# XMUDM/SPEX

Measured on AMD Instinct MI355X. Metric: graph-conv edges/sec + BPR-triples/sec, LightGCN-SPEX Epinion2 d=64, higher is better.
Workload: dtype f32

## Files before the change

### include/spex_hip.h

```cpp
#ifndef SPEX_HIP_H
#define SPEX_HIP_H

#include <stdint.h>

#ifdef __cplusplus
extern "C" {
#endif

typedef enum spex_status {
    SPEX_OK = 0,
    SPEX_ERR_INVALID = -1,
    SPEX_ERR_HIP = -2,
    SPEX_ERR_COMM = -3,
    SPEX_ERR_UNSUPPORTED = -4
} spex_status;

typedef struct spex_graph spex_graph_t;

int spex_version(void);
const char *spex_last_error(void);

int spex_graph_create(const int32_t *h_rowptr, const int32_t *h_col, const float *h_val, const int32_t *h_edge_id,
                      int32_t n_rows, int32_t n_cols, int64_t nnz, spex_graph_t **out);
int spex_graph_destroy(spex_graph_t *g);
int spex_graph_pack_digest(const int32_t *h_rowptr, const int32_t *h_col, const float *h_val, int32_t n_rows, int32_t n_cols,
                           int64_t nnz, uint64_t *digest );
int spex_graph_pack_hub_table(const int32_t *h_rowptr, const int32_t *h_col, const float *h_val, int32_t n_rows, int32_t n_cols,
                              int64_t nnz, int32_t *out, int64_t cap, int64_t *n_out);
int spex_graph_pack_row_heads(const int32_t *h_rowptr, const int32_t *h_col, const float *h_val, int32_t n_rows, int32_t n_cols,
                              int64_t nnz, int32_t *out_col, float *out_val, int64_t cap, int64_t *n_out, int32_t *stride);
int spex_graph_info(const spex_graph_t *g, int32_t *n_rows, int32_t *n_cols, int64_t *nnz, int32_t *n_long_rows,
                    int32_t *n_segments);

int spex_graph_set_edge_mask(spex_graph_t *g, int mode , const uint8_t *d_keep,
                             float keep_prob, uint64_t seed);

int spex_spmm_f32(const spex_graph_t *g, const float *X, float *Y, const float *add_in, float add_div,
                  const float *acc_in, float *acc_out, float acc_div, int32_t d, void *stream);

int spex_spmm_rowlist_f32(const spex_graph_t *g, const float *X, const int64_t *idx_a, int32_t n_a, int64_t off_a,
                          const int64_t *idx_b, int32_t n_b, int64_t off_b, float *Y, const float *acc_in, float *acc_out,
                          float acc_div, int32_t d, void *stream);
int spex_spmm_owned_rows_f32(const spex_graph_t *g, const float *X, const int64_t *pos, int32_t n, int64_t lo, const float *acc_in,
                             const float *acc2, const float *acc3, float acc_div, const float *raw, float *out_prop, float *out_raw,
                             int32_t d, void *stream);

int spex_propagate_f32(const spex_graph_t *g, const float *E0, float *mean_out, float *layers_out, float *ws,
                       int32_t L, int32_t d, void *stream);

int spex_propagate_bwd_f32(const spex_graph_t *gt, const float *g_out, float *grad_E0, float *ws, int32_t L,
                           int32_t d, void *stream);

int spex_cast_bf16_f32(const float *X, uint16_t *X16, int64_t n, void *stream);

int spex_spmm_bf16_f32(const spex_graph_t *g, const uint16_t *X16, float *Y, uint16_t *Y16, const float *add_in, float add_div,
// ... 430 lines not shown
```

### spex_amd/_lib.py

```python
import ctypes
import os

_HERE = os.path.dirname(os.path.abspath(__file__))
LIB_PATH = os.path.join(_HERE, "lib", "libspexhip.so")

c_i32, c_i64, c_f32, c_vp = ctypes.c_int32, ctypes.c_int64, ctypes.c_float, ctypes.c_void_p

SIGNATURES = {
    "spex_version": (ctypes.c_int, []),
    "spex_last_error": (ctypes.c_char_p, []),
    "spex_graph_create": (ctypes.c_int, [c_vp, c_vp, c_vp, c_vp, c_i32, c_i32, c_i64, ctypes.POINTER(c_vp)]),
    "spex_graph_destroy": (ctypes.c_int, [c_vp]),
    "spex_graph_pack_digest": (ctypes.c_int, [c_vp, c_vp, c_vp, c_i32, c_i32, c_i64, c_vp]),
    "spex_graph_pack_hub_table": (ctypes.c_int, [c_vp, c_vp, c_vp, c_i32, c_i32, c_i64, c_vp, c_i64, c_vp]),
    "spex_graph_pack_row_heads": (ctypes.c_int, [c_vp, c_vp, c_vp, c_i32, c_i32, c_i64, c_vp, c_vp, c_i64, c_vp, c_vp]),
    "spex_graph_info": (ctypes.c_int, [c_vp, ctypes.POINTER(c_i32), ctypes.POINTER(c_i32), ctypes.POINTER(c_i64),
                                       ctypes.POINTER(c_i32), ctypes.POINTER(c_i32)]),
    "spex_graph_set_edge_mask": (ctypes.c_int, [c_vp, ctypes.c_int, c_vp, c_f32, ctypes.c_uint64]),
    "spex_spmm_f32": (ctypes.c_int, [c_vp, c_vp, c_vp, c_vp, c_f32, c_vp, c_vp, c_f32, c_i32, c_vp]),
    "spex_spmm_rowlist_f32": (ctypes.c_int, [c_vp, c_vp, c_vp, c_i32, c_i64, c_vp, c_i32, c_i64, c_vp, c_vp, c_vp, c_f32, c_i32,
                                             c_vp]),
    "spex_spmm_owned_rows_f32": (ctypes.c_int, [c_vp, c_vp, c_vp, c_i32, c_i64, c_vp, c_vp, c_vp, c_f32, c_vp, c_vp, c_vp, c_i32, c_vp]),
    "spex_propagate_f32": (ctypes.c_int, [c_vp, c_vp, c_vp, c_vp, c_vp, c_i32, c_i32, c_vp]),
    "spex_propagate_bwd_f32": (ctypes.c_int, [c_vp, c_vp, c_vp, c_vp, c_i32, c_i32, c_vp]),
    "spex_cast_bf16_f32": (ctypes.c_int, [c_vp, c_vp, c_i64, c_vp]),
    "spex_spmm_bf16_f32": (ctypes.c_int, [c_vp, c_vp, c_vp, c_vp, c_vp, c_f32, c_vp, c_vp, c_f32, c_i32, c_vp]),
    "spex_propagate_bf16_f32": (ctypes.c_int, [c_vp, c_vp, c_vp, c_vp, c_i32, c_i32, c_vp]),
    "spex_propagate_bwd_bf16_f32": (ctypes.c_int, [c_vp, c_vp, c_vp, c_vp, c_vp, c_i32, c_i32, c_vp]),
    "spex_score_bce_f32": (ctypes.c_int, [c_vp, c_vp, c_i32, c_i32, c_i64, c_i64, c_vp, c_vp, c_vp, c_i32, c_i32, c_vp,
                                          c_vp, c_vp, c_vp, c_f32, c_vp]),
    "spex_score_bce_slots_f32": (ctypes.c_int, [c_vp, c_vp, c_i32, c_i32, c_i64, c_i64, c_vp, c_vp, c_vp, c_i32, c_i32, c_vp, c_vp,
                                                c_vp, c_f32, c_vp, c_i32, c_vp]),
    "spex_bpr_sgd_step_f32": (ctypes.c_int, [c_vp, c_vp, c_vp, c_vp, c_i64, c_i64, c_vp, c_vp, c_vp, c_i64, c_i32,
                                             c_f32, c_f32, c_vp, c_vp]),
    "spex_bpr_loss_f32": (ctypes.c_int, [c_vp, c_vp, c_i64, c_i64, c_vp, c_vp, c_vp, c_i64, c_i32, c_vp, c_vp, c_vp,
                                         c_f32, c_vp]),
    "spex_bpr_grouped_workspace_bytes": (c_i64, [c_i64, c_i64, c_i64]),
    "spex_bpr_sgd_step_grouped_f32": (ctypes.c_int, [c_vp, c_vp, c_vp, c_vp, c_i64, c_i64, c_vp, c_vp, c_vp, c_i64, c_i32,
                                                     c_f32, c_f32, c_vp, c_vp, c_i64, c_vp]),
    "spex_bpr_loss_grouped_f32": (ctypes.c_int, [c_vp, c_vp, c_i64, c_i64, c_vp, c_vp, c_vp, c_i64, c_i32, c_vp, c_vp, c_vp,
# ... 253 lines not shown
```

### spex_amd/csrc/graph.hip

```cpp
#include <stdarg.h>
#include <stdio.h>

#include <stdlib.h>

#include <algorithm>
#include <string>
#include <thread>
#include <vector>

#include "spex_common.h"

namespace spex {
static thread_local char g_err[512] = "";
void set_error(const char *fmt, ...)
{
    va_list ap;
    va_start(ap, fmt);
    vsnprintf(g_err, sizeof(g_err), fmt, ap);
    va_end(ap);
}
}

extern "C" int spex_version(void) { return 5; }
extern "C" const char *spex_last_error(void) { return spex::g_err; }
// ... 177 lines not shown
            long_seg0.push_back((int32_t)seg_beg.size());
            for (int32_t s = b; s < e; s += spex::kSegLen) {
                seg_beg.push_back(s);
                seg_end.push_back(s + spex::kSegLen < e ? s + spex::kSegLen : e);
            }
        }
    }
    long_seg0.push_back((int32_t)seg_beg.size());
    g->n_long = (int32_t)long_row.size();
    g->n_seg = (int32_t)seg_beg.size();

    std::vector<int4> task;
    std::vector<uint32_t> c_off, c_mask, c_eid;
    std::vector<uint8_t> c_pad;
    std::vector<int32_t> c_row;
    std::vector<float> c_val;
    std::vector<int32_t> hub_row, hub_seg0;
    std::vector<int4> hub_grp;
    std::vector<int2> hub_fold;
    const bool chunked = true;
    const char *implied_sw = getenv("SPEX_PACK_IMPLIED");
    const bool pack_implied = !(implied_sw && implied_sw[0] == '0');
    g->row_ids = (int64_t)n_cols * 256 <= ((int64_t)16 << 20);
    (void)flags;
    const int32_t tile_rows = 0;
    std::vector<int32_t> wg_rows;
    constexpr int kResidentWgs = 512;
    int open_tasks_now = spex::kOpenTasks;
    int pack_cap = spex::kTaskEntries;
    bool final_pass = false;
    for (int attempt = 0; chunked && attempt < 12; ++attempt) {
        task.clear();
        wg_rows.clear();
        hub_row.clear();
        hub_seg0.clear();
        hub_grp.clear();
        hub_fold.clear();
        struct ChunkJob { int64_t first_chunk; int64_t rows_off; int32_t n_rows, b, e, r0; };
        std::vector<ChunkJob> jobs;
        std::vector<int32_t> pack_rows;
        int64_t n_planned = 0;
        jobs.reserve((size_t)nnz / 48 + 64);
        pack_rows.reserve((size_t)n_rows + 64);
        auto add_chunks = [&](const int32_t *rows, int32_t n_rows_in, int32_t b, int32_t e, int32_t r0) -> int2 {
            int64_t entries = 0;
            ChunkJob j{n_planned, (int64_t)pack_rows.size(), 0, b, e, r0};
// ... 26 lines not shown
            for (const int4 &t : task)
                if (t.y > stride) return;
            std::vector<int64_t> moved(jobs.size(), -1);
            for (size_t k = 0; k < task.size(); ++k) {
                int4 &t = task[k];
                if (t.y > 0) {
                    const size_t j = (size_t)(std::lower_bound(jobs.begin(), jobs.end(), (int64_t)t.x,
                                                               [](const ChunkJob &jb, int64_t v) { return jb.first_chunk < v; }) - jobs.begin());
                    moved[j] = (int64_t)k * stride;
                }
                t.x = (int32_t)((int64_t)k * stride);
            }
            for (size_t j = 0; j < jobs.size(); ++j) jobs[j].first_chunk = moved[j];
            n_planned = (int64_t)task.size() * stride;
            implied = true;
            g->chunk_stride = stride;
        };
        auto fill_chunks = [&]() {
            place_implied();
            const size_t n_slots = (size_t)n_planned * spex::kChunk;
            c_off.resize(n_slots);
            c_val.resize(n_slots);
            c_eid.resize(n_slots);
            if (g->row_ids) c_row.resize(n_slots);
            c_mask.resize((size_t)n_planned);
            c_pad.assign((size_t)n_planned, implied ? (uint8_t)spex::kChunk : (uint8_t)0);
            const bool row_ids = g->row_ids;
            auto fill_job = [&](const ChunkJob &j) {
                size_t pos = (size_t)j.first_chunk * spex::kChunk, ci = (size_t)j.first_chunk;
                int32_t in_chunk = 0, last_col = 0, last_eid = 0, last_row = j.r0;
                uint32_t mask = 0;
                auto put = [&](int32_t en, int32_t r, bool last) {
                    last_col = h_col[en];
                    last_eid = h_edge_id ? h_edge_id[en] : en;
                    last_row = r;
                    c_off[pos] = (uint32_t)last_col;
                    c_val[pos] = h_val[en];
                    c_eid[pos] = (uint32_t)last_eid;
                    if (row_ids) c_row[pos] = r;
                    ++pos;
                    if (last) mask |= 1u << in_chunk;
                    if (++in_chunk == spex::kChunk) {
                        c_mask[ci] = mask;
                        c_pad[ci++] = 0;
                        mask = 0;
                        in_chunk = 0;
                    }
                };
                if (j.n_rows < 0) {
                    const int32_t n = -j.n_rows, nch = (n + spex::kChunk - 1) / spex::kChunk;
                    for (int32_t k = 0; k < nch * spex::kChunk; ++k, ++pos) {
                        c_off[pos] = 0u;
                        c_val[pos] = 0.0f;
                        c_eid[pos] = 0u;
                        if (row_ids) c_row[pos] = pack_rows[(size_t)j.rows_off + (k < n ? k : n - 1)];
                    }
                    for (int32_t c = 0; c < nch; ++c) {
                        c_mask[ci + c] = 0u;
                        c_pad[ci + c] = (uint8_t)spex::kChunk;
                    }
                    return;
                }
                if (j.n_rows) {
                    for (int32_t i = 0; i < j.n_rows; ++i) {
                        const int32_t r = pack_rows[(size_t)j.rows_off + i];
                        for (int32_t en = h_rowptr[r]; en < h_rowptr[r + 1]; ++en) put(en, r, en + 1 == h_rowptr[r + 1]);
                    }
                } else {
                    for (int32_t en = j.b; en < j.e; ++en) put(en, j.r0, false);
                }
                if (in_chunk) {
                    const uint32_t n_pad = (uint32_t)(spex::kChunk - in_chunk);
                    for (; in_chunk < spex::kChunk; ++in_chunk, ++pos) {
                        c_off[pos] = (uint32_t)last_col;
                        c_val[pos] = 0.0f;
                        c_eid[pos] = (uint32_t)last_eid;
                        if (row_ids) c_row[pos] = last_row;
                    }
                    c_mask[ci] = mask;
                    c_pad[ci] = (uint8_t)n_pad;
                }
            };
            std::vector<size_t> cut((size_t)n_thr + 1, jobs.size());
            cut[0] = 0;
            for (int p = 1; p < n_thr; ++p) {
                const int64_t want = n_planned * p / n_thr;
                if (implied) {
                    cut[p] = jobs.size() * (size_t)p / (size_t)n_thr;
                    continue;
                }
                cut[p] = (size_t)(std::lower_bound(jobs.begin(), jobs.end(), want,
                                                   [](const ChunkJob &j, int64_t v) { return j.first_chunk < v; }) - jobs.begin());
            }
            parallel_parts(n_thr, [&](int p) {
                for (size_t k = cut[p]; k < cut[p + 1]; ++k) fill_job(jobs[k]);
            });
        };
// ... 154 lines not shown
    }
    g->n_tasks = (int32_t)task.size();
    g->tile_rows = tile_rows;
    g->n_wgs = (int32_t)wg_rows.size();
    std::vector<int32_t> head_col;
    std::vector<float> head_val;
    {
        const char *heads_sw = getenv("SPEX_ROW_HEADS");
        const bool wanted = !digest || head_col_dump;
        if (wanted && g->row_ids && hub_row.empty() && nnz > 0 && !(heads_sw && heads_sw[0] == '0')) {
            head_col.assign((size_t)n_rows * spex::kRowHead, 0);
            head_val.assign((size_t)n_rows * spex::kRowHead, 0.0f);
            parallel_parts(n_thr, [&](int p) {
                const int32_t r_lo = (int32_t)((int64_t)n_rows * p / n_thr), r_hi = (int32_t)((int64_t)n_rows * (p + 1) / n_thr);
                for (int32_t r = r_lo; r < r_hi; ++r) {
                    const int32_t b = h_rowptr[r], n = std::min(h_rowptr[r + 1] - b, (int32_t)spex::kRowHead);
                    std::copy(h_col + b, h_col + b + n, head_col.begin() + (size_t)r * spex::kRowHead);
                    std::copy(h_val + b, h_val + b + n, head_val.begin() + (size_t)r * spex::kRowHead);
                }
            });
        }
    }
    if (getenv("SPEX_DEBUG_PACK"))
        fprintf(stderr, "[spex] graph %d x %d nnz %lld: %d tasks = %d workgroups, %lld chunks (%.1f %% padding), tile mode %d (%d workgroups), chunk stride %d, chunk table %lld bytes, row heads %lld bytes\n",
                n_rows, n_cols, (long long)nnz, (int)task.size(), (int)task.size() / spex::kWgWaves, (long long)c_mask.size(),
                nnz ? 100.0 * ((double)c_mask.size() * spex::kChunk - (double)nnz) / (double)nnz : 0.0, tile_rows, g->n_wgs, g->chunk_stride,
                (long long)(c_off.size() * 4 + c_val.size() * 4 + c_eid.size() * 4 + c_row.size() * 4 + c_mask.size() * 4 + c_pad.size()),
                (long long)(head_col.size() * 4 + head_val.size() * 4));
    g->n_chunks = (int64_t)c_mask.size();
    g->n_hub = (int32_t)hub_row.size();
    g->n_hub_tasks = (int32_t)hub_grp.size();

    g->tile = (nnz / spex::kSoftmaxTile < 2048) ? 512 : spex::kSoftmaxTile;
    g->n_tiles = (int32_t)((nnz + g->tile - 1) / g->tile);
    std::vector<int32_t> tile_row((size_t)g->n_tiles + 1);
    {
        int32_t r = 0;
        for (int32_t t = 0; t <= g->n_tiles; ++t) {
            const int64_t first = (int64_t)t * g->tile;
            while (r < n_rows && (int64_t)h_rowptr[r] < first) ++r;
            tile_row[t] = r;
        }
    }

    if (digest) {
        if (hub_dump) {
            hub_dump->clear();
            hub_dump->push_back((int32_t)hub_grp.size());
            hub_dump->push_back((int32_t)hub_fold.size());
            for (size_t k = 0; k < hub_grp.size(); ++k) {
                const int4 t = task[k], q = hub_grp[k];
// ... 56 lines not shown
        hipError_t e = hipMalloc((void **)&g->partial, (size_t)g->partial_cap * sizeof(float));
        if (e != hipSuccess) {
            spex::set_error("hipMalloc(partial) failed: %s", hipGetErrorString(e));
            spex_graph_destroy(g);
            return SPEX_ERR_HIP;
        }
    }
    *out = g;
    return SPEX_OK;
}

extern "C" int spex_graph_info(const spex_graph_t *g, int32_t *n_rows, int32_t *n_cols, int64_t *nnz,
                               int32_t *n_long_rows, int32_t *n_segments)
{
    SPEX_CHECK_ARG(g, "spex_graph_info: NULL handle");
    if (n_rows) *n_rows = g->n_rows;
    if (n_cols) *n_cols = g->n_cols;
    if (nnz) *nnz = g->nnz;
    if (n_long_rows) *n_long_rows = g->n_long;
    if (n_segments) *n_segments = g->n_seg;
    return SPEX_OK;
}

extern "C" int spex_graph_set_edge_mask(spex_graph_t *g, int mode, const uint8_t *d_keep, float keep_prob,
                                        uint64_t seed)
{
    SPEX_CHECK_ARG(g, "spex_graph_set_edge_mask: NULL handle");
    SPEX_CHECK_ARG(mode >= 0 && mode <= 2, "spex_graph_set_edge_mask: mode %d not in {0,1,2}", mode);
    SPEX_CHECK_ARG(mode != 1 || d_keep, "spex_graph_set_edge_mask: injected mode needs a device mask");
    SPEX_CHECK_ARG(mode == 0 || (keep_prob > 0.0f), "spex_graph_set_edge_mask: keep_prob must be > 0");
    if (mode != 0 && keep_prob >= 1.0f && mode == 2) mode = 0;
    g->mask_mode = mode;
    g->keep = (mode == 1) ? d_keep : nullptr;
    g->keep_prob = keep_prob;
    g->seed = seed;
    return SPEX_OK;
}

extern "C" int spex_timer_create(int32_t capacity, int32_t every, spex_timer_t **out)
{
    SPEX_CHECK_ARG(out && capacity > 0 && capacity <= (1 << 20), "spex_timer_create: bad capacity %d", capacity);
    SPEX_CHECK_ARG(every >= 1, "spex_timer_create: every = %d", every);
    spex_timer *t = new spex_timer();
    t->every = every;
    t->start.resize(capacity);
    t->stop.resize(capacity);
// ... 45 lines not shown
```

### spex_amd/csrc/spex_common.h

```cpp
#pragma once
#include <hip/hip_runtime.h>
#include <stdint.h>
#include <mutex>
#include <string>
#include <vector>

#include "../../include/spex_hip.h"

namespace spex {

void set_error(const char *fmt, ...);
struct SmallAdam {
    float *p = nullptr, *m = nullptr, *v = nullptr;
    const float *parts = nullptr;
    int32_t n_parts = 0;
    int64_t stride = 0;
    int32_t n = 0;
};
struct L2Rows {
    const int32_t *count = nullptr;
    int32_t *clear = nullptr;
    float scale = 0.0f;
    float *g_store = nullptr;
    int32_t shift = 4;
// ... 280 lines not shown
    int32_t *seg_end = nullptr;
    int32_t *long_row = nullptr;
    int32_t *long_seg0 = nullptr;
    float *partial = nullptr;
    int64_t partial_cap = 0;
    float *snap = nullptr;
    int64_t snap_cap = 0;
    unsigned long long *loss_cell = nullptr;
    int64_t loss_cell_cap = 0;
    std::mutex scratch_mu;
    hipStream_t scratch_stream = nullptr;
    bool scratch_used = false;
    hipEvent_t scratch_ev = nullptr;
    int32_t n_tasks = 0;
    int4 *task = nullptr;
    int64_t n_chunks = 0;
    uint32_t *chunk_off = nullptr;
    float *chunk_val = nullptr;
    uint32_t *chunk_mask = nullptr;
    uint8_t *chunk_pad = nullptr;
    uint32_t *chunk_eid = nullptr;
    bool row_ids = false;
    int32_t *chunk_row = nullptr;
    int32_t chunk_stride = 0;
    int32_t *head_col = nullptr;
    float *head_val = nullptr;
    int32_t tile_rows = 0;
    int32_t n_wgs = 0;
    int32_t *wg_rows = nullptr;
    int32_t n_hub = 0;
    int32_t *hub_row = nullptr;
    int32_t *hub_seg0 = nullptr;
    int32_t n_hub_tasks = 0;
    int4 *hub_grp = nullptr;
    int2 *hub_fold = nullptr;
    unsigned long long *hub_ticket = nullptr;
    int mask_mode = 0;
    const uint8_t *keep = nullptr;
    float keep_prob = 1.0f;
    uint64_t seed = 0;
    spex_timer *timer = nullptr;
};
```

### spex_amd/csrc/spmm.hip

```cpp
#include <mutex>

#include "spmm_chunk.h"

using namespace spex;
using namespace spex::chunkk;

namespace {

struct SpmmParams {
    const int32_t *rowptr, *col;
    const float *val;
    const int32_t *edge_id;
    const int32_t *seg_beg, *seg_end, *long_row, *long_seg0;
    int32_t n_rows, n_seg, n_long;

    const float *X;
    float *Y;
    const float *add_in;
    float add_div;
    float out_div;
    const float *acc_in;
    float *acc_out;
    float acc_div;
    float *partial;
// ... 147 lines not shown
template <int V>
struct VecOf {
    typedef float T __attribute__((ext_vector_type(V)));
};

template <int EPI, bool MASKED, bool ROWIDS, int V>
__global__ __launch_bounds__(kWave *kWgWaves) void spmm_chunk_wide_kernel(
    const float *__restrict__ X, const uint32_t *__restrict__ chunk_off, const float *__restrict__ chunk_val,
    const uint32_t *__restrict__ chunk_mask, const int32_t *__restrict__ chunk_row, const int4 *__restrict__ task,
    int n_tasks, float *__restrict__ Y,
    const float *epi_in, float epi_div, float out_div, float *acc_out,
    float *__restrict__ partial,
    const DropArgs drop, const int xcd_contiguous)
{
    typedef typename VecOf<V>::T vec;
    constexpr int kRow = kWave * V;
    constexpr int kBatch = kChunk / V;
    __shared__ float s_part[kWgWaves][kRow];
    const int lane = threadIdx.x & (kWave - 1);
    const int wave = __builtin_amdgcn_readfirstlane((int)(threadIdx.x >> 6));
    const int wg = xcd_contiguous ? xcd_contiguous_block(blockIdx.x, gridDim.x) : (int)blockIdx.x;
    const int tid = wg * kWgWaves + wave;
    if (tid >= n_tasks) return;
    const int4 t = task[tid];
    const int kind = t.w & 3;
    const float *__restrict__ Xl = X + lane * V;
    const float *El = (EPI ? epi_in : X) + lane * V;
    int row = t.z;
    vec acc = (vec)(0.0f);

    auto emit = [&](int r, vec y, vec e) {
        const size_t o = (size_t)r * kRow + lane * V;
        if (EPI == 0) {
            __builtin_nontemporal_store(y, reinterpret_cast<vec *>(Y + o));
        } else if (EPI == 1) {
            if (Y) __builtin_nontemporal_store(y, reinterpret_cast<vec *>(Y + o));
            vec s = e + y;
            if (epi_div != 1.0f) s = s / epi_div;
            __builtin_nontemporal_store(s, reinterpret_cast<vec *>(acc_out + o));
        } else {
            if (epi_div != 1.0f) e = e / epi_div;
            vec s = y + e;
            if (out_div != 1.0f) s = s / out_div;
            __builtin_nontemporal_store(s, reinterpret_cast<vec *>(Y + o));
        }
    };

    const int n_ch = kind == 3 ? 0 : t.y;
    for (int sc = 0; sc < n_ch; sc += 4) {
        const int nc = (n_ch - sc < 4) ? n_ch - sc : 4;
        uint32_t my_off = 0u, my_mask = 0u, own_off = 0u;
        unsigned long long drop_bits = 0ull;
        int my_row = 0;
        float my_val = 0.0f;
        if (lane < nc * kChunk) {
            const size_t e = (size_t)(t.x + sc) * kChunk + lane;
            my_off = __builtin_nontemporal_load(chunk_off + e);
            my_val = __builtin_nontemporal_load(chunk_val + e);
            if (ROWIDS) my_row = __builtin_nontemporal_load(chunk_row + e);
            if (MASKED) own_off = drop_lane(drop, __builtin_nontemporal_load(drop.chunk_eid + e), my_val, my_off);
        }
        if (MASKED) drop_bits = drop_stand_in(lane < nc * kChunk, own_off, my_off);
        if (lane < nc) my_mask = __builtin_nontemporal_load(chunk_mask + t.x + sc + lane);
        for (int c = 0; c < nc; ++c) {
            const uint32_t mask = (uint32_t)__builtin_amdgcn_readlane((int)my_mask, c);
            const uint32_t dbits = MASKED ? (uint32_t)(drop_bits >> (c * kChunk)) & 0xFFFFu : 0u;
#pragma unroll
            for (int u0 = 0; u0 < kChunk; u0 += kBatch) {
                vec x[kBatch], ep[kBatch];
#pragma unroll
                for (int u = 0; u < kBatch; ++u)
                    x[u] = *reinterpret_cast<const vec *>(
                        Xl + (size_t)(uint32_t)__builtin_amdgcn_readlane((int)my_off, c * kChunk + u0 + u) * kRow);
                const uint32_t bmask = (mask >> u0) & ((1u << kBatch) - 1u);
                if (EPI != 0 && bmask != 0u) {
                    int r = row;
#pragma unroll
                    for (int u = 0; u < kBatch; ++u) {
                        ep[u] = (vec)(0.0f);
                        if (bmask & (1u << u)) {
                            const int rr = ROWIDS ? __builtin_amdgcn_readlane(my_row, c * kChunk + u0 + u) : r;
                            ep[u] = __builtin_nontemporal_load(reinterpret_cast<const vec *>(El + (size_t)rr * kRow));
                            ++r;
                        }
                    }
                } else {
// ... 2 lines not shown
                }
#pragma unroll
                for (int u = 0; u < kBatch; ++u) {
                    const float a = lane_bcast(my_val, c * kChunk + u0 + u);
                    const bool gone = MASKED && (dbits & (1u << (u0 + u)));
#pragma unroll
                    for (int j = 0; j < V; ++j) acc[j] = fmaf(a, gone ? 0.0f : x[u][j], acc[j]);
                    if (bmask & (1u << u)) {
                        emit(ROWIDS ? __builtin_amdgcn_readlane(my_row, c * kChunk + u0 + u) : row, acc, ep[u]);
                        acc = (vec)(0.0f);
                        ++row;
                    }
                }
            }
        }
    }
    if (kind == 0 && t.y == 0 && t.z >= 0) {
        vec e = (vec)(0.0f);
        if (EPI != 0) e = *reinterpret_cast<const vec *>(El + (size_t)t.z * kRow);
        emit(t.z, (vec)(0.0f), e);
    }
    if (ROWIDS && kind == 3) {
        const int count = t.w >> 4;
        const int my_r = lane < count ? chunk_row[(size_t)t.x * kChunk + lane] : 0;
        for (int k0 = 0; k0 < count; k0 += kBatch) {
            vec e[kBatch];
#pragma unroll
            for (int u = 0; u < kBatch; ++u) {
                e[u] = (vec)(0.0f);
                if (EPI != 0 && k0 + u < count) e[u] = *reinterpret_cast<const vec *>(El + (size_t)__builtin_amdgcn_readlane(my_r, (k0 + u) & 63) * kRow);
            }
#pragma unroll
            for (int u = 0; u < kBatch; ++u)
                if (k0 + u < count) emit(__builtin_amdgcn_readlane(my_r, (k0 + u) & 63), (vec)(0.0f), e[u]);
        }
    }
    if (kind == 2) {
#pragma unroll
        for (int j = 0; j < V; ++j) partial[(size_t)(t.w >> 4) * kRow + lane * V + j] = acc[j];
    }
    if (t.w & 4) {
        const bool leader = kind == 1 && (t.w & 8);
        const int slot = (t.w >> 4) & 15, nseg = (t.w >> 8) & 31;
        vec e = (vec)(0.0f);
        if (leader && EPI != 0) e = *reinterpret_cast<const vec *>(El + (size_t)t.z * kRow);
        if (kind == 1 && !leader) {
#pragma unroll
// ... 334 lines not shown
    const int per_block = fast ? kWgWaves : kWavesPerBlock;
    const int64_t tasks = fast ? (int64_t)g->n_tasks : (int64_t)g->n_seg + g->n_rows;
    int64_t blocks = (tasks + per_block - 1) / per_block;
    blocks = (blocks + 7) / 8 * 8;
    SnapArgs sa{nullptr, nullptr, nullptr, nullptr, 0, 0, 0, (int32_t)blocks};
    int64_t tail = 0;
    if (snap) {
        SPEX_CHECK_ARG(fast && d == 64 && !masked && !acc_out && !add_in && snap->out && snap->T > 0, "launch_spmm: the snapshot tail rides on the plain d == 64 launch only");
        sa = *snap;
        sa.table_wgs = (int32_t)blocks;
        tail = (3 * snap->T + (int64_t)kWgWaves * kWave - 1) / ((int64_t)kWgWaves * kWave);
    }
    const dim3 grid((unsigned)(blocks + tail)), block(kWave * per_block), block4(kWave * kWavesPerBlock);
    spex_timer *tm = g->timer;
    if (tm && tm->open) tm->launches[tm->used]++;
    std::unique_lock<std::mutex> scratch_lock;
    if ((fast ? g->n_hub > 0 : g->n_long > 0) || snap) {
        const int rc = order_scratch(g, stream, scratch_lock);
        if (rc) return rc;
    }
    if (fast) {
        SPEX_CHECK_ARG(((((uintptr_t)X) | ((uintptr_t)Y) | ((uintptr_t)add_in) | ((uintptr_t)acc_in) | ((uintptr_t)acc_out)) & 15) == 0,
                       "spex_spmm_f32: X / Y / add_in / acc_in / acc_out must be 16-byte aligned");
        const int xcd_contig = ((int64_t)g->n_cols * d * 4 <= (int64_t)16 << 20) ? 1 : 0;
        const DropArgs da = drop_args(g);
        const char *fold_sw = g->n_hub > 0 ? getenv("SPEX_HUB_FOLD") : nullptr;
        const bool fold_env = !(fold_sw && fold_sw[0] == '0');
        hub.grp = g->hub_grp; hub.fold = g->hub_fold; hub.ticket = g->hub_ticket;
        hub.tag = (d == 64 && fold_env && g->n_hub > 0 && g->hub_grp && g->hub_ticket) ? 1u : 0u;
        if (acc_out) launch_chunk<1>(d, masked, g->row_ids, grid, block, stream, X, g, Y, acc_in, acc_div, 1.0f, acc_out, da, xcd_contig, hub, sa);
        else if (add_in) launch_chunk<2>(d, masked, g->row_ids, grid, block, stream, X, g, Y, add_in, add_div, out_div, nullptr, da, xcd_contig, hub, sa);
        else launch_chunk<0>(d, masked, g->row_ids, grid, block, stream, X, g, Y, nullptr, 1.0f, 1.0f, nullptr, da, xcd_contig, hub, sa);
    } else if (masked) {
        hipLaunchKernelGGL((spmm_rows_kernel<true>), grid, block, 0, stream, p);
    } else {
        hipLaunchKernelGGL((spmm_rows_kernel<false>), grid, block, 0, stream, p);
    }
    if (fast) {
        if (g->n_hub > 0 && hub.tag == 0u) {
            const dim3 fgrid((unsigned)((g->n_hub + kWavesPerBlock - 1) / kWavesPerBlock));
            hipLaunchKernelGGL(spmm_long_fixup_kernel, fgrid, block4, 0, stream, p, g->hub_row, g->hub_seg0, g->hub_seg0 + 1, 2,
                               g->n_hub);
        }
    } else if (g->n_long > 0) {
        const dim3 fgrid((unsigned)((g->n_long + kWavesPerBlock - 1) / kWavesPerBlock));
        hipLaunchKernelGGL(spmm_long_fixup_kernel, fgrid, block4, 0, stream, p, g->long_row, g->long_seg0, g->long_seg0 + 1, 1,
// ... 262 lines not shown
```

### spex_amd/csrc/spmm_bf16.hip

```cpp
#include <mutex>

#include "spmm_chunk.h"

using namespace spex;
using namespace spex::chunkk;

namespace {

template <int EPI, bool MASKED, bool ROWIDS>
__global__ __launch_bounds__(kWave *kWgWaves) __attribute__((amdgpu_waves_per_eu(8, 8))) void spmm_chunk_bf16_kernel(
    const uint16_t *__restrict__ X16, const uint32_t *__restrict__ chunk_off, const float *__restrict__ chunk_val,
    const uint32_t *__restrict__ chunk_mask, const int32_t *__restrict__ chunk_row, const int4 *__restrict__ task,
    int n_tasks, float *__restrict__ Y, uint16_t *__restrict__ Y16,
    const float *epi_in, float epi_div, float *acc_out,
    float *__restrict__ partial, const DropArgs drop, const int xcd_contiguous, const int chunk_stride)
{
    chunk_body<uint16_t, EPI, MASKED, ROWIDS, false>(chunk_off, chunk_val, chunk_row, chunk_mask, task, n_tasks, xcd_contiguous, chunk_stride,
                                                     0, X16, Y, ChunkSide<uint16_t>{Y16}, epi_in, epi_div, acc_out, partial, drop,
                                                     HubFold{nullptr, nullptr, nullptr, 0u}, SnapArgs{});
}


__global__ __launch_bounds__(kWave *kWavesPerBlock) void spmm_hub_fixup_bf16_kernel(
    const float *__restrict__ partial, const int32_t *__restrict__ rows, const int32_t *__restrict__ seg, int n_hub,
// ... 65 lines not shown
    hipLaunchKernelGGL((spmm_chunk_bf16_kernel<EPI, M, R>), grid, block, 0, stream, X16, g->chunk_off, g->chunk_val, g->chunk_mask, \
                       g->chunk_row, g->task, g->n_tasks, Y, Y16, epi_in, epi_div, acc_out, g->partial, da, xcd_contig, g->chunk_stride)
    if (masked) {
        if (row_ids) SPEX_GO(true, true);
        else SPEX_GO(true, false);
    } else {
        if (row_ids) SPEX_GO(false, true);
        else SPEX_GO(false, false);
    }
#undef SPEX_GO
}

int launch_spmm_bf16(const spex_graph *g, const uint16_t *X16, float *Y, uint16_t *Y16, const float *add_in, float add_div,
                     const float *acc_in, float *acc_out, float acc_div, hipStream_t stream)
{
    if (g->n_rows == 0) return SPEX_OK;
    const bool masked = g->mask_mode != 0;
    const dim3 grid((unsigned)chunk_table_wgs(g)), block(kWave * kWgWaves);
    std::unique_lock<std::mutex> scratch_lock;
    if (g->n_hub > 0) {
        const int rc = order_scratch(g, stream, scratch_lock);
        if (rc) return rc;
    }
    const int xcd_contig = ((int64_t)g->n_cols * 64 * 2 <= (int64_t)16 << 20) ? 1 : 0;
    const DropArgs da = drop_args(g);
    if (acc_out) launch_chunk_bf16<1>(masked, g->row_ids, grid, block, stream, X16, g, Y, Y16, acc_in, acc_div, acc_out, da, xcd_contig);
    else if (add_in) launch_chunk_bf16<2>(masked, g->row_ids, grid, block, stream, X16, g, Y, Y16, add_in, add_div, nullptr, da, xcd_contig);
    else launch_chunk_bf16<0>(masked, g->row_ids, grid, block, stream, X16, g, Y, Y16, nullptr, 1.0f, nullptr, da, xcd_contig);
    if (g->n_hub > 0) {
        const dim3 fgrid((unsigned)((g->n_hub + kWavesPerBlock - 1) / kWavesPerBlock));
        hipLaunchKernelGGL(spmm_hub_fixup_bf16_kernel, fgrid, dim3(kWave * kWavesPerBlock), 0, stream, g->partial, g->hub_row, g->hub_seg0,
                           g->n_hub, Y, Y16, add_in, add_div, acc_in, acc_out, acc_div);
    }
    SPEX_HIP(hipGetLastError());
    return SPEX_OK;
}

bool aligned16(const void *a, const void *b = nullptr, const void *c = nullptr, const void *d = nullptr, const void *e = nullptr,
               const void *f = nullptr)
{
    return ((((uintptr_t)a) | ((uintptr_t)b) | ((uintptr_t)c) | ((uintptr_t)d) | ((uintptr_t)e) | ((uintptr_t)f)) & 15) == 0;
}

int check_graph_bf16(const spex_graph *g, const char *who, bool square)
{
    SPEX_CHECK_ARG(!square || g->n_rows == g->n_cols, "%s: needs a square graph (%d x %d)", who, g->n_rows, g->n_cols);
// ... 124 lines not shown
```

### spex_amd/csrc/spmm_chunk.h

```cpp
#pragma once
#include "spex_common.h"

namespace spex {
namespace chunkk {

__device__ __forceinline__ int xcd_contiguous_block(int bid, int nblk)
{
    return ((nblk & 7) == 0) ? (bid & 7) * (nblk >> 3) + (bid >> 3) : bid;
}

inline int64_t chunk_table_wgs(const spex_graph *g)
{
    return (((int64_t)g->n_tasks + kWgWaves - 1) / kWgWaves + 7) / 8 * 8;
}

#ifndef SPEX_EPI_NT
#define SPEX_EPI_NT 1
#endif
#if SPEX_EPI_NT
#define SPEX_EPI_LOAD(p) __builtin_nontemporal_load(p)
#else
#define SPEX_EPI_LOAD(p) (*(p))
#endif

// ... 164 lines not shown
    const int chunk_stride, const int table_wgs,
    const XT *__restrict__ X, float *__restrict__ Y, const ChunkSide<XT> side,
    const float *epi_in, float epi_div, float *acc_out,
    float *__restrict__ partial, const DropArgs &drop, const HubFold &hf_args, const SnapArgs &snap)
{
    typedef Gather16<XT> G;
    __shared__ float s_part[kWgWaves][kWave];
    const int lane = threadIdx.x & (kWave - 1);
    const int wave = __builtin_amdgcn_readfirstlane((int)(threadIdx.x >> 6));
    constexpr bool kTail = EPI == 0 && !MASKED && FOLD;
    if constexpr (kTail) {
        if ((int)blockIdx.x >= table_wgs) {
            const int64_t slot0 = ((int64_t)((int)blockIdx.x - table_wgs) * kWgWaves + wave) * kWave;
            if (slot0 < 3 * snap.T) snapshot_rows(snap, X, slot0, lane);
            return;
        }
    }
    constexpr bool kFront = sizeof(XT) == 4;
    const int n_wg = kFront ? (kTail ? table_wgs : (int)gridDim.x) : 0;
    const int wg = xcd_contiguous ? xcd_contiguous_block(blockIdx.x, kFront ? n_wg : (int)gridDim.x) : (int)blockIdx.x;
    const int tid = wg * kWgWaves + wave;
    if (tid >= n_tasks) return;
    const bool implied = ROWIDS && chunk_stride != 0;
    uint32_t pre_off = 0u, pre_mask = 0u, pre_eid = 0u;
    int pre_row = 0;
    float pre_val = 0.0f;
    if (implied) {
        const size_t c0 = (size_t)tid * (size_t)chunk_stride, e = c0 * kChunk + lane;
        pre_off = __builtin_nontemporal_load(chunk_off + e);
        pre_val = __builtin_nontemporal_load(chunk_val + e);
        pre_row = __builtin_nontemporal_load(chunk_row + e);
        if (MASKED) pre_eid = __builtin_nontemporal_load(drop.chunk_eid + e);
        pre_mask = __builtin_nontemporal_load(chunk_mask + c0 + (lane & 3));
    }
    const int4 t = task[tid];
    const int kind = t.w & 3;
    const XT *__restrict__ Xl = X + lane;
    const float *El = epi_in + lane;
    int row = t.z;
    float acc = 0.0f;

    const float epi_inv = 1.0f / epi_div;
    auto emit = [&](int r, float y, float e) {
        const size_t o = (size_t)r * 64 + lane;
        if (EPI == 0) {
            put<false>(Y, side, o, y);
        } else if (EPI == 1) {
            const float s = scaled(e + y, epi_div, epi_inv);
            put<true>(Y, side, o, y);
            __builtin_nontemporal_store(s, acc_out + o);
        } else {
            put<false>(Y, side, o, finish(side, y + scaled(e, epi_div, epi_inv)));
        }
    };

    if (ROWIDS && kind == 3) {
        const int count = t.w >> 4;
        int my_r = -1;
        if (lane < count) my_r = implied ? pre_row : chunk_row[(size_t)t.x * kChunk + lane];
        const int sub = lane & 15, grp = lane >> 4;
        const f4 zero = (f4)(0.0f);
        for (int k0 = 0; k0 < count; k0 += 16) {
            int r[4];
            f4 e[4];
#pragma unroll
            for (int j = 0; j < 4; ++j) {
                r[j] = __shfl(my_r, (k0 + 4 * j + grp) & 63, kWave);
                if (k0 + 4 * j + grp >= count) r[j] = -1;
                e[j] = zero;
                if (EPI != 0 && r[j] >= 0) e[j] = *reinterpret_cast<const f4 *>(epi_in + (size_t)r[j] * 64 + sub * 4);
            }
#pragma unroll
            for (int j = 0; j < 4; ++j) {
                if (r[j] < 0) continue;
                const size_t o = (size_t)r[j] * 64 + sub * 4;
                if (EPI == 0) {
                    put<false>(Y, side, o, zero);
                } else if (EPI == 1) {
                    f4 sv = e[j] + zero;
                    if (epi_div != 1.0f) sv = sv / epi_div;
                    put<true>(Y, side, o, zero);
                    __builtin_nontemporal_store(sv, reinterpret_cast<f4 *>(acc_out + o));
// ... 6 lines not shown
        }
    }
    const int n_ch = kind == 3 ? 0 : t.y;
    auto super_chunk = [&](const int sc, const bool first) __attribute__((always_inline)) {
        const int nc = (n_ch - sc < 4) ? n_ch - sc : 4;
        uint32_t my_off = 0u, my_mask = 0u, own_off = 0u;
        unsigned long long drop_bits = 0ull;
        int my_row = 0;
        float my_val = 0.0f;
        if (lane < nc * kChunk) {
            uint32_t eid = 0u;
            if (first) {
                my_off = pre_off;
                my_val = pre_val;
                my_row = pre_row;
                if (MASKED) eid = pre_eid;
            } else {
                const size_t e = (size_t)(t.x + sc) * kChunk + lane;
                my_off = __builtin_nontemporal_load(chunk_off + e);
                my_val = __builtin_nontemporal_load(chunk_val + e);
                if (ROWIDS) my_row = __builtin_nontemporal_load(chunk_row + e);
                if (MASKED) eid = __builtin_nontemporal_load(drop.chunk_eid + e);
            }
            if (MASKED) own_off = drop_lane(drop, eid, my_val, my_off);
        }
        if (MASKED) drop_bits = drop_stand_in(lane < nc * kChunk, own_off, my_off);
        if (first) my_mask = pre_mask;
        else if (lane < nc) my_mask = __builtin_nontemporal_load(chunk_mask + t.x + sc + lane);
        float ep[kChunk];
#pragma unroll
        for (int u = 0; u < kChunk; ++u) ep[u] = 0.0f;
        for (int c = 0; c < nc; ++c) {
            const uint32_t mask = (uint32_t)__builtin_amdgcn_readlane((int)my_mask, c);
            const uint32_t dbits = MASKED ? (uint32_t)(drop_bits >> (c * kChunk)) & 0xFFFFu : 0u;
            typename G::R x[kChunk / G::kPer];
#pragma unroll
            for (int u = 0; u < kChunk; ++u)
                x[u >> G::kShift] = reg_with(x[u >> G::kShift], u & (G::kPer - 1), Xl[(size_t)(uint32_t)__builtin_amdgcn_readlane((int)my_off, c * kChunk + u) * 64]);
            if (EPI != 0 && mask != 0u) {
                int r = row;
#pragma unroll
                for (int u = 0; u < kChunk; ++u) {
                    if (mask & (1u << u)) {
                        const int rr = ROWIDS ? __builtin_amdgcn_readlane(my_row, c * kChunk + u) : r;
                        ep[u] = SPEX_EPI_LOAD(El + (size_t)rr * 64);
                        ++r;
// ... 8 lines not shown
                    acc = fmaf(lane_bcast(my_val, c * kChunk + u), xv, acc);
                }
                continue;
            }
#pragma unroll
            for (int u = 0; u < kChunk; ++u) {
                const float xv = (MASKED && (dbits & (1u << u))) ? 0.0f : reg_value(x[u >> G::kShift], u & (G::kPer - 1));
                acc = fmaf(lane_bcast(my_val, c * kChunk + u), xv, acc);
                if (mask & (1u << u)) {
                    emit(ROWIDS ? __builtin_amdgcn_readlane(my_row, c * kChunk + u) : row, acc, ep[u]);
                    acc = 0.0f;
                    ++row;
                }
            }
        }
    };
    if (ROWIDS) {
        if (n_ch > 0) {
            const int nc0 = n_ch < 4 ? n_ch : 4;
            if (!implied && lane < nc0 * kChunk) {
                const size_t e = (size_t)t.x * kChunk + lane;
                pre_off = __builtin_nontemporal_load(chunk_off + e);
                pre_val = __builtin_nontemporal_load(chunk_val + e);
                pre_row = __builtin_nontemporal_load(chunk_row + e);
                if (MASKED) pre_eid = __builtin_nontemporal_load(drop.chunk_eid + e);
                if (lane < nc0) pre_mask = __builtin_nontemporal_load(chunk_mask + t.x + lane);
            }
            super_chunk(0, true);
        }
        for (int sc = 4; sc < n_ch; sc += 4) super_chunk(sc, false);
    } else {
        for (int sc = 0; sc < n_ch; sc += 4) super_chunk(sc, false);
    }
    if (kind == 0 && t.y == 0 && t.z >= 0) {
        float e = 0.0f;
        if (EPI != 0) e = El[(size_t)t.z * 64];
        emit(t.z, 0.0f, e);
    }
    const bool hub = FOLD && kind == 2 && hf_args.tag != 0u;
    if (kind == 2 && !hub) partial[(size_t)(t.w >> 4) * 64 + lane] = acc;
    if (t.w & 4) {
        const bool leader = kind == 1 && (t.w & 8);
        const int slot = (t.w >> 4) & 15, nseg = (t.w >> 8) & 31;
        int4 hg = make_int4(0, 0, 0, 0);
        if (hub) hg = hf_args.grp[tid];
        const bool hub_leader = hub && hg.x != 0;
        float e = 0.0f;
// ... 44 lines not shown
```

### spex_amd/graph.py

```python
import ctypes

import numpy as np
import torch

from . import _lib


def bipartite_csr(users, items, n_u, n_i, self_loops=False, counts=False):
    key, mult = np.unique(np.asarray(users, np.int64) * np.int64(n_i) + np.asarray(items, np.int64), return_counts=True)
    uu, ii = key // n_i, key % n_i
    n = n_u + n_i
    rows = np.concatenate([uu, ii + n_u])
    cols = np.concatenate([ii + n_u, uu])
    mult = np.concatenate([mult, mult])
    if self_loops:
        eye = np.arange(n, dtype=np.int64)
        rows, cols, mult = np.concatenate([rows, eye]), np.concatenate([cols, eye]), np.concatenate([mult, np.ones(n, mult.dtype)])
    order = np.argsort(rows * np.int64(n) + cols, kind="stable")
    rows, cols, mult = rows[order], cols[order], mult[order]
    rowptr = np.zeros(n + 1, np.int64)
    np.cumsum(np.bincount(rows, minlength=n), out=rowptr[1:])
    out = (rowptr.astype(np.int32), rows.astype(np.int32), cols.astype(np.int32))
    return out + (mult,) if counts else out

# ... 104 lines not shown
class SpexGraph:

    def __init__(self, rowptr, col, val, n_cols=None, edge_id=None, device=None):
        rowptr = np.ascontiguousarray(rowptr, np.int32)
        col = np.ascontiguousarray(col, np.int32)
        val = np.ascontiguousarray(val, np.float32)
        self.n_rows = len(rowptr) - 1
        self.n_cols = int(n_cols if n_cols is not None else self.n_rows)
        self.nnz = int(len(col))
        self.host = (rowptr, col, val)
        if edge_id is not None:
            edge_id = np.ascontiguousarray(edge_id, np.int32)
        self._edge_id_host = edge_id
        self.device = _device_of(device)
        handle = ctypes.c_void_p()
        with torch.cuda.device(self.device):
            args = (rowptr.ctypes.data_as(ctypes.c_void_p), col.ctypes.data_as(ctypes.c_void_p), val.ctypes.data_as(ctypes.c_void_p),
                    edge_id.ctypes.data_as(ctypes.c_void_p) if edge_id is not None else None, self.n_rows, self.n_cols, self.nnz)
            _lib.call("spex_graph_create", *args, ctypes.byref(handle))
        self._h = handle
        nl, ns = ctypes.c_int32(), ctypes.c_int32()
        _lib.call("spex_graph_info", self._h, None, None, None, ctypes.byref(nl), ctypes.byref(ns))
        self.n_long_rows, self.n_segments = nl.value, ns.value
        self._mask_ref = None
        self.mask_mode = 0

    def size(self):
        return torch.Size([self.n_rows, self.n_cols])

    shape = property(size)

    def _nnz(self):
        return self.nnz

    def to_torch_sparse(self, device="cpu"):
        rowptr, col, val = self.host
        rows = np.repeat(np.arange(self.n_rows, dtype=np.int64), np.diff(rowptr))
        idx = torch.from_numpy(np.stack([rows, col.astype(np.int64)]))
        return torch.sparse_coo_tensor(idx, torch.from_numpy(val), (self.n_rows, self.n_cols)).coalesce().to(device)

    def close(self):
        if getattr(self, "_h", None) is not None and self._h.value:
            self.detach_timer()
            self.release_workspace()
            with torch.cuda.device(self.device):
                _lib.load().spex_graph_destroy(self._h)
# ... 229 lines not shown
```

Measured before the change: 36.28 billion.

## Pack row index into high half of chunk column offsets for small graphs

When the graph has at most 65536 rows and columns and uses row ids, each chunk entry's row index is stored in the upper 16 bits of the column-offset word. The separate chunk_row array is then not allocated, and the SpMM kernels decode row and column from a single load. This removes one 4-byte stream per edge from the gather loop in exchange for a shift and mask. It only applies when task chunk counts stay at or below 4 and the pack capacity is the default, and launch checks guard that invariant. It also adds a layout query API.

```diff
diff --git a/include/spex_hip.h b/include/spex_hip.h
--- a/include/spex_hip.h
+++ b/include/spex_hip.h
@@ -31,6 +31,7 @@
                               int64_t nnz, int32_t *out_col, float *out_val, int64_t cap, int64_t *n_out, int32_t *stride);
 int spex_graph_info(const spex_graph_t *g, int32_t *n_rows, int32_t *n_cols, int64_t *nnz, int32_t *n_long_rows,
                     int32_t *n_segments);
+int spex_graph_layout(const spex_graph_t *g, int32_t *bin_packed, int32_t *packed_words, int32_t *chunk_stride);
 
 int spex_graph_set_edge_mask(spex_graph_t *g, int mode , const uint8_t *d_keep,
                              float keep_prob, uint64_t seed);
diff --git a/spex_amd/_lib.py b/spex_amd/_lib.py
--- a/spex_amd/_lib.py
+++ b/spex_amd/_lib.py
@@ -16,6 +16,7 @@
     "spex_graph_pack_row_heads": (ctypes.c_int, [c_vp, c_vp, c_vp, c_i32, c_i32, c_i64, c_vp, c_vp, c_i64, c_vp, c_vp]),
     "spex_graph_info": (ctypes.c_int, [c_vp, ctypes.POINTER(c_i32), ctypes.POINTER(c_i32), ctypes.POINTER(c_i64),
                                        ctypes.POINTER(c_i32), ctypes.POINTER(c_i32)]),
+    "spex_graph_layout": (ctypes.c_int, [c_vp, ctypes.POINTER(c_i32), ctypes.POINTER(c_i32), ctypes.POINTER(c_i32)]),
     "spex_graph_set_edge_mask": (ctypes.c_int, [c_vp, ctypes.c_int, c_vp, c_f32, ctypes.c_uint64]),
     "spex_spmm_f32": (ctypes.c_int, [c_vp, c_vp, c_vp, c_vp, c_f32, c_vp, c_vp, c_f32, c_i32, c_vp]),
     "spex_spmm_rowlist_f32": (ctypes.c_int, [c_vp, c_vp, c_vp, c_i32, c_i64, c_vp, c_i32, c_i64, c_vp, c_vp, c_vp, c_f32, c_i32,
diff --git a/spex_amd/csrc/graph.hip b/spex_amd/csrc/graph.hip
--- a/spex_amd/csrc/graph.hip
+++ b/spex_amd/csrc/graph.hip
@@ -223,6 +223,8 @@
     const char *implied_sw = getenv("SPEX_PACK_IMPLIED");
     const bool pack_implied = !(implied_sw && implied_sw[0] == '0');
     g->row_ids = (int64_t)n_cols * 256 <= ((int64_t)16 << 20);
+    const char *words_sw = getenv("SPEX_PACK_WORDS");
+    g->packed_words = g->row_ids && n_rows <= 65536 && n_cols <= 65536 && !(words_sw && words_sw[0] == '0');
     (void)flags;
     const int32_t tile_rows = 0;
     std::vector<int32_t> wg_rows;
@@ -295,10 +297,15 @@
             c_off.resize(n_slots);
             c_val.resize(n_slots);
             c_eid.resize(n_slots);
-            if (g->row_ids) c_row.resize(n_slots);
+            if (pack_cap != spex::kTaskEntries) g->packed_words = false;
+            for (const int4 &t : task)
+                if ((t.w & 3) != 3 && t.y > g->max_task_chunks) g->max_task_chunks = t.y;
+            if (g->max_task_chunks > 4) g->packed_words = false;
+            const bool packed = g->packed_words;
+            if (g->row_ids && !packed) c_row.resize(n_slots);
             c_mask.resize((size_t)n_planned);
             c_pad.assign((size_t)n_planned, implied ? (uint8_t)spex::kChunk : (uint8_t)0);
-            const bool row_ids = g->row_ids;
+            const bool row_ids = g->row_ids && !packed;
             auto fill_job = [&](const ChunkJob &j) {
                 size_t pos = (size_t)j.first_chunk * spex::kChunk, ci = (size_t)j.first_chunk;
                 int32_t in_chunk = 0, last_col = 0, last_eid = 0, last_row = j.r0;
@@ -307,7 +314,7 @@
                     last_col = h_col[en];
                     last_eid = h_edge_id ? h_edge_id[en] : en;
                     last_row = r;
-                    c_off[pos] = (uint32_t)last_col;
+                    c_off[pos] = packed ? ((uint32_t)r << 16) | (uint32_t)last_col : (uint32_t)last_col;
                     c_val[pos] = h_val[en];
                     c_eid[pos] = (uint32_t)last_eid;
                     if (row_ids) c_row[pos] = r;
@@ -323,10 +330,11 @@
                 if (j.n_rows < 0) {
                     const int32_t n = -j.n_rows, nch = (n + spex::kChunk - 1) / spex::kChunk;
                     for (int32_t k = 0; k < nch * spex::kChunk; ++k, ++pos) {
-                        c_off[pos] = 0u;
+                        const int32_t r = pack_rows[(size_t)j.rows_off + (k < n ? k : n - 1)];
+                        c_off[pos] = packed ? (uint32_t)r << 16 : 0u;
                         c_val[pos] = 0.0f;
                         c_eid[pos] = 0u;
-                        if (row_ids) c_row[pos] = pack_rows[(size_t)j.rows_off + (k < n ? k : n - 1)];
+                        if (row_ids) c_row[pos] = r;
                     }
                     for (int32_t c = 0; c < nch; ++c) {
                         c_mask[ci + c] = 0u;
@@ -345,7 +353,7 @@
                 if (in_chunk) {
                     const uint32_t n_pad = (uint32_t)(spex::kChunk - in_chunk);
                     for (; in_chunk < spex::kChunk; ++in_chunk, ++pos) {
-                        c_off[pos] = (uint32_t)last_col;
+                        c_off[pos] = packed ? ((uint32_t)last_row << 16) | (uint32_t)last_col : (uint32_t)last_col;
                         c_val[pos] = 0.0f;
                         c_eid[pos] = (uint32_t)last_eid;
                         if (row_ids) c_row[pos] = last_row;
@@ -546,11 +554,12 @@
         }
     }
     if (getenv("SPEX_DEBUG_PACK"))
-        fprintf(stderr, "[spex] graph %d x %d nnz %lld: %d tasks = %d workgroups, %lld chunks (%.1f %% padding), tile mode %d (%d workgroups), chunk stride %d, chunk table %lld bytes, row heads %lld bytes\n",
+        fprintf(stderr, "[spex] graph %d x %d nnz %lld: %d tasks = %d workgroups, %lld chunks (%.1f %% padding), tile mode %d (%d workgroups), chunk stride %d, chunk table %lld bytes, row heads %lld bytes, %s\n",
                 n_rows, n_cols, (long long)nnz, (int)task.size(), (int)task.size() / spex::kWgWaves, (long long)c_mask.size(),
                 nnz ? 100.0 * ((double)c_mask.size() * spex::kChunk - (double)nnz) / (double)nnz : 0.0, tile_rows, g->n_wgs, g->chunk_stride,
                 (long long)(c_off.size() * 4 + c_val.size() * 4 + c_eid.size() * 4 + c_row.size() * 4 + c_mask.size() * 4 + c_pad.size()),
-                (long long)(head_col.size() * 4 + head_val.size() * 4));
+                (long long)(head_col.size() * 4 + head_val.size() * 4),
+                !g->row_ids ? "adjacent rows" : (g->packed_words ? "packed words" : "row array"));
     g->n_chunks = (int64_t)c_mask.size();
     g->n_hub = (int32_t)hub_row.size();
     g->n_hub_tasks = (int32_t)hub_grp.size();
@@ -653,6 +662,15 @@
     return SPEX_OK;
 }
 
+extern "C" int spex_graph_layout(const spex_graph_t *g, int32_t *bin_packed, int32_t *packed_words, int32_t *chunk_stride)
+{
+    SPEX_CHECK_ARG(g, "spex_graph_layout: NULL handle");
+    if (bin_packed) *bin_packed = g->row_ids ? 1 : 0;
+    if (packed_words) *packed_words = g->packed_words ? 1 : 0;
+    if (chunk_stride) *chunk_stride = g->chunk_stride;
+    return SPEX_OK;
+}
+
 extern "C" int spex_graph_set_edge_mask(spex_graph_t *g, int mode, const uint8_t *d_keep, float keep_prob,
                                         uint64_t seed)
 {
diff --git a/spex_amd/csrc/spex_common.h b/spex_amd/csrc/spex_common.h
--- a/spex_amd/csrc/spex_common.h
+++ b/spex_amd/csrc/spex_common.h
@@ -326,6 +326,8 @@
     uint32_t *chunk_eid = nullptr;
     bool row_ids = false;
     int32_t *chunk_row = nullptr;
+    bool packed_words = false;
+    int32_t max_task_chunks = 0;
     int32_t chunk_stride = 0;
     int32_t *head_col = nullptr;
     float *head_val = nullptr;
diff --git a/spex_amd/csrc/spmm.hip b/spex_amd/csrc/spmm.hip
--- a/spex_amd/csrc/spmm.hip
+++ b/spex_amd/csrc/spmm.hip
@@ -193,6 +193,7 @@
     const int wg = xcd_contiguous ? xcd_contiguous_block(blockIdx.x, gridDim.x) : (int)blockIdx.x;
     const int tid = wg * kWgWaves + wave;
     if (tid >= n_tasks) return;
+    const bool packed = ROWIDS && chunk_row == nullptr;
     const int4 t = task[tid];
     const int kind = t.w & 3;
     const float *__restrict__ Xl = X + lane * V;
@@ -228,11 +229,17 @@
             const size_t e = (size_t)(t.x + sc) * kChunk + lane;
             my_off = __builtin_nontemporal_load(chunk_off + e);
             my_val = __builtin_nontemporal_load(chunk_val + e);
-            if (ROWIDS) my_row = __builtin_nontemporal_load(chunk_row + e);
-            if (MASKED) own_off = drop_lane(drop, __builtin_nontemporal_load(drop.chunk_eid + e), my_val, my_off);
+            if (ROWIDS && !packed) my_row = __builtin_nontemporal_load(chunk_row + e);
+            uint32_t eid = 0u;
+            if (MASKED) eid = __builtin_nontemporal_load(drop.chunk_eid + e);
+            if (lane < nc) my_mask = __builtin_nontemporal_load(chunk_mask + t.x + sc + lane);
+            if (packed) {
+                my_row = (int)(my_off >> 16);
+                my_off &= 0xFFFFu;
+            }
+            if (MASKED) own_off = drop_lane(drop, eid, my_val, my_off);
         }
         if (MASKED) drop_bits = drop_stand_in(lane < nc * kChunk, own_off, my_off);
-        if (lane < nc) my_mask = __builtin_nontemporal_load(chunk_mask + t.x + sc + lane);
         for (int c = 0; c < nc; ++c) {
             const uint32_t mask = (uint32_t)__builtin_amdgcn_readlane((int)my_mask, c);
             const uint32_t dbits = MASKED ? (uint32_t)(drop_bits >> (c * kChunk)) & 0xFFFFu : 0u;
@@ -281,7 +288,8 @@
     }
     if (ROWIDS && kind == 3) {
         const int count = t.w >> 4;
-        const int my_r = lane < count ? chunk_row[(size_t)t.x * kChunk + lane] : 0;
+        int my_r = 0;
+        if (lane < count) my_r = packed ? (int)(chunk_off[(size_t)t.x * kChunk + lane] >> 16) : chunk_row[(size_t)t.x * kChunk + lane];
         for (int k0 = 0; k0 < count; k0 += kBatch) {
             vec e[kBatch];
 #pragma unroll
@@ -662,6 +670,7 @@
     if (fast) {
         SPEX_CHECK_ARG(((((uintptr_t)X) | ((uintptr_t)Y) | ((uintptr_t)add_in) | ((uintptr_t)acc_in) | ((uintptr_t)acc_out)) & 15) == 0,
                        "spex_spmm_f32: X / Y / add_in / acc_in / acc_out must be 16-byte aligned");
+        SPEX_CHECK_ARG(!(g->packed_words && g->max_task_chunks > 4), "spex_spmm_f32: packed words on a table with tasks of %d chunks", g->max_task_chunks);
         const int xcd_contig = ((int64_t)g->n_cols * d * 4 <= (int64_t)16 << 20) ? 1 : 0;
         const DropArgs da = drop_args(g);
         const char *fold_sw = g->n_hub > 0 ? getenv("SPEX_HUB_FOLD") : nullptr;
diff --git a/spex_amd/csrc/spmm_bf16.hip b/spex_amd/csrc/spmm_bf16.hip
--- a/spex_amd/csrc/spmm_bf16.hip
+++ b/spex_amd/csrc/spmm_bf16.hip
@@ -111,6 +111,7 @@
         const int rc = order_scratch(g, stream, scratch_lock);
         if (rc) return rc;
     }
+    SPEX_CHECK_ARG(!(g->packed_words && g->max_task_chunks > 4), "spex_spmm_bf16_f32: packed words on a table with tasks of %d chunks", g->max_task_chunks);
     const int xcd_contig = ((int64_t)g->n_cols * 64 * 2 <= (int64_t)16 << 20) ? 1 : 0;
     const DropArgs da = drop_args(g);
     if (acc_out) launch_chunk_bf16<1>(masked, g->row_ids, grid, block, stream, X16, g, Y, Y16, acc_in, acc_div, acc_out, da, xcd_contig);
diff --git a/spex_amd/csrc/spmm_chunk.h b/spex_amd/csrc/spmm_chunk.h
--- a/spex_amd/csrc/spmm_chunk.h
+++ b/spex_amd/csrc/spmm_chunk.h
@@ -210,6 +210,13 @@
     const int tid = wg * kWgWaves + wave;
     if (tid >= n_tasks) return;
     const bool implied = ROWIDS && chunk_stride != 0;
+    auto is_packed = [&]() __attribute__((always_inline)) {
+        if (!ROWIDS) return false;
+        unsigned long long p = (unsigned long long)chunk_row;
+        asm volatile("" : "+s"(p));
+        return p == 0ull;
+    };
+    const bool packed = is_packed();
     uint32_t pre_off = 0u, pre_mask = 0u, pre_eid = 0u;
     int pre_row = 0;
     float pre_val = 0.0f;
@@ -217,7 +224,7 @@
         const size_t c0 = (size_t)tid * (size_t)chunk_stride, e = c0 * kChunk + lane;
         pre_off = __builtin_nontemporal_load(chunk_off + e);
         pre_val = __builtin_nontemporal_load(chunk_val + e);
-        pre_row = __builtin_nontemporal_load(chunk_row + e);
+        if (!packed) pre_row = __builtin_nontemporal_load(chunk_row + e);
         if (MASKED) pre_eid = __builtin_nontemporal_load(drop.chunk_eid + e);
         pre_mask = __builtin_nontemporal_load(chunk_mask + c0 + (lane & 3));
     }
@@ -245,7 +252,10 @@
     if (ROWIDS && kind == 3) {
         const int count = t.w >> 4;
         int my_r = -1;
-        if (lane < count) my_r = implied ? pre_row : chunk_row[(size_t)t.x * kChunk + lane];
+        if (lane < count) {
+            if (packed) my_r = (int)((implied ? pre_off : chunk_off[(size_t)t.x * kChunk + lane]) >> 16);
+            else my_r = implied ? pre_row : chunk_row[(size_t)t.x * kChunk + lane];
+        }
         const int sub = lane & 15, grp = lane >> 4;
         const f4 zero = (f4)(0.0f);
         for (int k0 = 0; k0 < count; k0 += 16) {
@@ -298,6 +308,10 @@
                 if (ROWIDS) my_row = __builtin_nontemporal_load(chunk_row + e);
                 if (MASKED) eid = __builtin_nontemporal_load(drop.chunk_eid + e);
             }
+            if (first && is_packed()) {
+                my_row = (int)(my_off >> 16);
+                my_off &= 0xFFFFu;
+            }
             if (MASKED) own_off = drop_lane(drop, eid, my_val, my_off);
         }
         if (MASKED) drop_bits = drop_stand_in(lane < nc * kChunk, own_off, my_off);
@@ -352,7 +366,7 @@
                 const size_t e = (size_t)t.x * kChunk + lane;
                 pre_off = __builtin_nontemporal_load(chunk_off + e);
                 pre_val = __builtin_nontemporal_load(chunk_val + e);
-                pre_row = __builtin_nontemporal_load(chunk_row + e);
+                if (!packed) pre_row = __builtin_nontemporal_load(chunk_row + e);
                 if (MASKED) pre_eid = __builtin_nontemporal_load(drop.chunk_eid + e);
                 if (lane < nc0) pre_mask = __builtin_nontemporal_load(chunk_mask + t.x + lane);
             }
diff --git a/spex_amd/graph.py b/spex_amd/graph.py
--- a/spex_amd/graph.py
+++ b/spex_amd/graph.py
@@ -150,6 +150,9 @@
         nl, ns = ctypes.c_int32(), ctypes.c_int32()
         _lib.call("spex_graph_info", self._h, None, None, None, ctypes.byref(nl), ctypes.byref(ns))
         self.n_long_rows, self.n_segments = nl.value, ns.value
+        bp, pw, cs = ctypes.c_int32(), ctypes.c_int32(), ctypes.c_int32()
+        _lib.call("spex_graph_layout", self._h, ctypes.byref(bp), ctypes.byref(pw), ctypes.byref(cs))
+        self.bin_packed, self.packed_words, self.chunk_stride = bool(bp.value), bool(pw.value), cs.value
         self._mask_ref = None
         self.mask_mode = 0
 
```

Result: faster. 36.72 billion, median of 6 (+1.2%).
